# pyprob/pyprob

Measured on NVIDIA H100. Metric: ic_train_traces_per_sec, higher is better.
Workload: dtype f32

## Files before the change

### pyprob_b200/csrc/obs_embed.inc

```

struct ObsLayout {
  int in_off[PPB_MAX_OBS], out_off[PPB_MAX_OBS];
  int max_depth;
};
inline ObsLayout obs_layout(const ppb_net_desc& D) {
  ObsLayout o;
  int ci = 0, co = 0;
  o.max_depth = 0;
  for (int j = 0; j < D.num_obs; ++j) {
    o.in_off[j] = ci; o.out_off[j] = co;
    ci += D.obs_ff[j].in_dim; co += D.obs_ff[j].out_dim;
    o.max_depth = D.obs_ff[j].num_layers > o.max_depth ? D.obs_ff[j].num_layers : o.max_depth;
  }
  return o;
}

template <class W>
void obs_fp32_plan_fwd(Builder& bl, const ppb_net_desc& D, const float* arena, const float* obs, int B, const W& w,
                       float* obs_emb) {
  const int E = D.obs_dim;
  const ObsLayout o = obs_layout(D);
  for (int l = 0; l < o.max_depth; ++l) {
    bl.begin();
    for (int j = 0; j < D.num_obs; ++j) {
      const ppb_ff_desc& ff = D.obs_ff[j];
      if (l >= ff.num_layers) continue;
      const ppb_linear_desc& L = ff.layers[l];
      const float* X = l == 0 ? obs + o.in_off[j] : w.obs_act[j][l - 1];
      int64_t ldx = l == 0 ? D.obs_in_total : ff.layers[l - 1].out_dim;
      bool last = (l == ff.num_layers - 1);
      float* Y = last ? w.obs_cat + o.out_off[j] : w.obs_act[j][l];
      int64_t ldy = last ? E : L.out_dim;
      bl.add(linear_fwd(X, ldx, arena + L.w_off, L.in_dim, arena + L.b_off, Y, ldy, B, L.out_dim, L.in_dim, gemm::kRelu));
    }
  }
  for (int l = 0; l < D.obs_final.num_layers; ++l) {
    bl.begin();
    const ppb_linear_desc& L = D.obs_final.layers[l];
    const float* X = l == 0 ? w.obs_cat : w.fin_act[l - 1];
    bool last = (l == D.obs_final.num_layers - 1);
    float* Y = last ? obs_emb : w.fin_act[l];
    bl.add(linear_fwd(X, L.in_dim, arena + L.w_off, L.in_dim, arena + L.b_off, Y, L.out_dim, B, L.out_dim, L.in_dim, gemm::kRelu));
  }
}

inline int obs_bias_grad(const ppb_linear_desc& L, const float* dY, int64_t ld, int B, float* grad, cudaStream_t st) {
  k_colsum_gather<<<dim3((L.out_dim + 31) / 32, 8), 256, 0, st>>>(dY, ld, nullptr, B, L.out_dim, grad + L.b_off);
  PPB_LAUNCH_CHECK();
  return PPB_OK;
}

int obs_fp32_plan_bwd(Builder& bl, const ppb_net_desc& D, const float* arena, float* grad, const float* obs, int B,
                      const Ws& w) {
  const int E = D.obs_dim;
  const int first = (int)bl.phases.size();
  for (int l = D.obs_final.num_layers - 1; l >= 0; --l) {
    const ppb_linear_desc& L = D.obs_final.layers[l];
    const float* X = l == 0 ? w.obs_cat : w.fin_act[l - 1];
    float* dY = (l == D.obs_final.num_layers - 1) ? w.d_obs_emb : w.d_fin_act[l];
    float* dX = l == 0 ? w.d_obs_cat : w.d_fin_act[l - 1];
    bl.begin();
    bl.add(linear_dw(dY, L.out_dim, X, L.in_dim, grad + L.w_off, L.in_dim, B, L.out_dim, L.in_dim));
    Problem px = linear_dx(dY, L.out_dim, arena + L.w_off, L.in_dim, dX, L.in_dim, B, L.out_dim, L.in_dim, gemm::kMaskAux);
    px.aux = X; px.ld_aux = L.in_dim;
    bl.add(px);
  }
  const ObsLayout o = obs_layout(D);
  for (int l = o.max_depth - 1; l >= 0; --l) {
    bl.begin();
    for (int j = 0; j < D.num_obs; ++j) {
      const ppb_ff_desc& ff = D.obs_ff[j];
      if (l >= ff.num_layers) continue;
      const ppb_linear_desc& L = ff.layers[l];
      bool last = (l == ff.num_layers - 1);
      const float* X = l == 0 ? obs + o.in_off[j] : w.obs_act[j][l - 1];
      int64_t ldx = l == 0 ? D.obs_in_total : ff.layers[l - 1].out_dim;
      const float* dY = last ? w.d_obs_cat + o.out_off[j] : w.d_obs_act[j][l];
      int64_t lddy = last ? E : L.out_dim;
      bl.add(linear_dw(dY, lddy, X, ldx, grad + L.w_off, L.in_dim, B, L.out_dim, L.in_dim));
      if (l > 0) {
        Problem px = linear_dx(dY, lddy, arena + L.w_off, L.in_dim, w.d_obs_act[j][l - 1], ff.layers[l - 1].out_dim, B,
                               L.out_dim, L.in_dim, gemm::kMaskAux);
        px.aux = w.obs_act[j][l - 1]; px.ld_aux = ff.layers[l - 1].out_dim;
        bl.add(px);
      }
    }
  }
  return first;
}

int obs_fp32_bwd(const Builder& bl, int first, const Problem* dev, const ppb_net_desc& D, float* grad, int B, const Ws& w,
                 cudaStream_t st) {
  const int E = D.obs_dim;
  k_mask_nonpos<<<ew_grid((int64_t)B * E), 256, 0, st>>>(w.d_obs_emb, w.obs_emb, (int64_t)B * E);
  PPB_LAUNCH_CHECK();
  int ph = first, rc;
  for (int l = D.obs_final.num_layers - 1; l >= 0; --l) {
    const ppb_linear_desc& L = D.obs_final.layers[l];
    float* dY = (l == D.obs_final.num_layers - 1) ? w.d_obs_emb : w.d_fin_act[l];
    rc = obs_bias_grad(L, dY, L.out_dim, B, grad, st); if (rc) return rc;
    rc = run_phase(bl.phases[ph++], dev, st); if (rc) return rc;
  }
  const ObsLayout o = obs_layout(D);
  for (int l = o.max_depth - 1; l >= 0; --l) {
    for (int j = 0; j < D.num_obs; ++j) {
      const ppb_ff_desc& ff = D.obs_ff[j];
      if (l >= ff.num_layers) continue;
      const ppb_linear_desc& L = ff.layers[l];
      bool last = (l == ff.num_layers - 1);
      const float* dY = last ? w.d_obs_cat + o.out_off[j] : w.d_obs_act[j][l];
      rc = obs_bias_grad(L, dY, last ? E : L.out_dim, B, grad, st); if (rc) return rc;
    }
    rc = run_phase(bl.phases[ph++], dev, st); if (rc) return rc;
  }
  return PPB_OK;
}

inline obsmlp::Plan obs_plan_of(const ppb_net_desc& D, const Ws* w, const float* obs) {
  obsmlp::Plan P;
  memset(&P, 0, sizeof(P));
  const int E = D.obs_dim;
  const ObsLayout lay = obs_layout(D);
  P.E = E;
  int nf = 0;
  auto add_layer = [&](const ppb_linear_desc& L) -> obsmlp::Layer& {
    obsmlp::Layer& o = P.L[P.n_layers++];
    o.in_dim = L.in_dim; o.out_dim = L.out_dim; o.w_off = L.w_off; o.b_off = L.b_off;
    o.pitch = (L.in_dim & 3) ? L.in_dim : ((L.in_dim & 7) ? L.in_dim : L.in_dim + 4);
    o.sw = nf;
    nf += (L.out_dim * o.pitch + L.out_dim + 3) & ~3;
    o.part = P.part_floats;
    P.part_floats += L.out_dim * L.in_dim + L.out_dim;
    return o;
  };
  std::vector<int> first(D.num_obs);
  for (int j = 0; j < D.num_obs; ++j) {
    const ppb_ff_desc& ff = D.obs_ff[j];
    first[j] = P.n_layers;
    for (int l = 0; l < ff.num_layers; ++l) {
      obsmlp::Layer& o = add_layer(ff.layers[l]);
      o.xoff = P.A; P.A += o.in_dim;
      if (l + 1 < ff.num_layers) { o.dzoff = P.Dz; P.Dz += o.out_dim; }
      o.dxoff = l == 0 ? -1 : P.L[P.n_layers - 2].dzoff;
      o.x = l == 0 ? obs + lay.in_off[j] : (w ? w->obs_act[j][l - 1] : nullptr);
      o.ldx = l == 0 ? D.obs_in_total : ff.layers[l - 1].out_dim;
      if (l + 1 < ff.num_layers) { o.y = w ? w->obs_act[j][l] : nullptr; o.ldy = o.out_dim; }
    }
  }
  const int cat = P.A, dcat = P.Dz;
  P.A += E; P.Dz += E;
  for (int j = 0; j < D.num_obs; ++j) {
    obsmlp::Layer& o = P.L[first[j] + D.obs_ff[j].num_layers - 1];
    o.yoff = cat + lay.out_off[j]; o.dzoff = dcat + lay.out_off[j];
    o.y = w ? w->obs_cat + lay.out_off[j] : nullptr; o.ldy = E;
  }
  for (int j = 0; j < D.num_obs; ++j)
    for (int l = 0; l + 1 < D.obs_ff[j].num_layers; ++l) P.L[first[j] + l].yoff = P.L[first[j] + l + 1].xoff;
  const int nfin = D.obs_final.num_layers;
  for (int l = 0; l < nfin; ++l) {
    const bool last = l == nfin - 1;
    obsmlp::Layer& o = add_layer(D.obs_final.layers[l]);
    if (l == 0) o.xoff = cat;
    o.yoff = P.A; P.A += o.out_dim;
    o.dzoff = P.Dz; P.Dz += o.out_dim;
    o.dxoff = l == 0 ? dcat : P.L[P.n_layers - 2].dzoff;
    o.x = l == 0 ? (w ? w->obs_cat : nullptr) : (w ? w->fin_act[l - 1] : nullptr);
    o.ldx = o.in_dim;
    o.y = w ? (last ? w->obs_emb : w->fin_act[l]) : nullptr; o.ldy = o.out_dim;
    if (l > 0) o.xoff = P.L[P.n_layers - 2].yoff;
  }
  P.w_floats = nf;
  return P;
}
inline bool obs_fused_ok(const ppb_net_desc& D) {
  constexpr int kFuseMaxWidth = obsmlp::W2;
  if (D.obs_dim > kFuseMaxWidth) return false;
  for (int j = 0; j < D.num_obs; ++j)
    for (int l = 0; l < D.obs_ff[j].num_layers; ++l)
      if (D.obs_ff[j].layers[l].in_dim > kFuseMaxWidth || D.obs_ff[j].layers[l].out_dim > kFuseMaxWidth) return false;
  for (int l = 0; l < D.obs_final.num_layers; ++l)
    if (D.obs_final.layers[l].in_dim > kFuseMaxWidth || D.obs_final.layers[l].out_dim > kFuseMaxWidth) return false;
  const obsmlp::Plan P = obs_plan_of(D, nullptr, nullptr);
  return obsmlp::smem_fwd(P) <= obsmlp::kMaxSmem && obsmlp::smem_bwd(P) <= obsmlp::kMaxSmem;
}
int obs_fused_fwd(const ppb_net_desc& D, const float* arena, const float* obs, int B, const Ws& w, cudaStream_t st,
                  const HImg* emb_img = nullptr) {
  int rc = smem_opt_in<obsmlp::k_fwd>(obsmlp::kMaxSmem);
  if (rc) return rc;
  obsmlp::Plan P = obs_plan_of(D, &w, obs);
  if (emb_img) {
    P.emb_k_hi = emb_img->k_hi; P.emb_k_lo = emb_img->k_lo; P.emb_mn_hi = emb_img->mn_hi; P.emb_mn_lo = emb_img->mn_lo;
    P.emb_kb = emb_img->kb;
  }
  const int tpc = (B + PPB_NUM_SMS - 1) / PPB_NUM_SMS;
  PPB_CUDA(ppb_launch(obsmlp::k_fwd, dim3((B + tpc - 1) / tpc), dim3(obsmlp::kThreads), obsmlp::smem_fwd(P), st, 1, 0, P, arena,
                      B, tpc));
  PPB_LAUNCH_CHECK();
  return PPB_OK;
}
int obs_fused_bwd(const ppb_net_desc& D, const float* arena, float* grad, const float* obs, int B, const Ws& w,
                  cudaStream_t st) {
  int rc = smem_opt_in<obsmlp::k_bwd>(obsmlp::kMaxSmem);
  if (rc) return rc;
  const obsmlp::Plan P = obs_plan_of(D, &w, obs);
  constexpr int kMaxCtas = 16 * obsmlp::kCluster;
  int tpc = (B + kMaxCtas - 1) / kMaxCtas;
  tpc = tpc < obsmlp::kMT ? obsmlp::kMT : tpc;
  int ctas = (B + tpc - 1) / tpc;
  ctas = (ctas + obsmlp::kCluster - 1) / obsmlp::kCluster * obsmlp::kCluster;
  PPB_CUDA(ppb_launch(obsmlp::k_bwd, dim3(ctas), dim3(obsmlp::kThreads), obsmlp::smem_bwd(P), st, 1, obsmlp::kCluster, P, arena,
                      (const float*)w.d_obs_emb, grad, B, tpc));
  PPB_LAUNCH_CHECK();
  return PPB_OK;
}

inline bool obs_tc_ok(const ppb_net_desc& D) {
  const ObsLayout o = obs_layout(D);
  for (int j = 0; j < D.num_obs; ++j) {
    const ppb_ff_desc& ff = D.obs_ff[j];
    if (ff.num_layers < 2 || (o.out_off[j] & 31)) return false;
    for (int l = 1; l < ff.num_layers; ++l)
      if (ff.layers[l].in_dim < 32) return false;
  }
  for (int l = 0; l < D.obs_final.num_layers; ++l)
    if (D.obs_final.layers[l].in_dim < 32) return false;
  return true;
}

template <class Add>
void obs_weight_images(ppb_net* net, Add add) {
  const ppb_net_desc& D = net->desc;
  net->obs_form = obs_fused_ok(D) ? ObsForm::fused : obs_tc_ok(D) ? ObsForm::tensor_core : ObsForm::simt;
  if (net->obs_form != ObsForm::tensor_core) return;
  for (int j = 0; j < D.num_obs; ++j)
    for (int l = 1; l < D.obs_ff[j].num_layers; ++l) {
      const ppb_linear_desc& L = D.obs_ff[j].layers[l];
      net->w_obs[j][l] = add(L.w_off, L.out_dim, L.in_dim, L.in_dim);
    }
  for (int l = 0; l < D.obs_final.num_layers; ++l) {
    const ppb_linear_desc& L = D.obs_final.layers[l];
    net->w_fin[l] = add(L.w_off, L.out_dim, L.in_dim, L.in_dim);
  }
}

struct ObsImgs {
  HImg act[PPB_MAX_OBS][PPB_MAX_FF_LAYERS], cat, fin[PPB_MAX_FF_LAYERS];
  HImg g_act[PPB_MAX_OBS][PPB_MAX_FF_LAYERS], g_cat, g_fin[PPB_MAX_FF_LAYERS], g_emb;
  char* begin; int64_t bytes;
};
template <class Img>
void obs_carve_images(const ppb_net* net, int B, Img img, ObsImgs& o) {
  if (net->obs_form != ObsForm::tensor_core) return;
  const ppb_net_desc& D = net->desc;
  for (int j = 0; j < D.num_obs; ++j)
    for (int l = 0; l + 1 < D.obs_ff[j].num_layers; ++l) {
      o.act[j][l] = img(B, D.obs_ff[j].layers[l].out_dim);
      o.g_act[j][l] = img(B, D.obs_ff[j].layers[l].out_dim);
    }
  o.cat = img(B, D.obs_dim);
  o.g_cat = img(B, D.obs_dim);
  for (int l = 0; l + 1 < D.obs_final.num_layers; ++l) {
    o.fin[l] = img(B, D.obs_final.layers[l].out_dim);
    o.g_fin[l] = img(B, D.obs_final.layers[l].out_dim);
  }
  o.g_emb = img(B, D.obs_dim);
}

__global__ void __launch_bounds__(256) k_pack_rows_masked(float* __restrict__ g, const float* __restrict__ y, int rows,
                                                           int cols, int64_t ld, HImg img) {
  ppb_pdl_trigger();
  ppb_pdl_wait();
  tc::pack_tile<tc::Parts::both>(blockIdx.x, (int)img.kb, img.k_hi, img.k_lo, img.mn_hi, img.mn_lo,
                                 [&](int row, int k0, float (&x)[4]) {
#pragma unroll
    for (int j = 0; j < 4; ++j) {
      x[j] = 0.0f;
      if (row < rows && k0 + j < cols) {
        const int64_t o = (int64_t)row * ld + k0 + j;
        x[j] = y[o] > 0.0f ? g[o] : 0.0f;
        g[o] = x[j];
      }
    }
  });
}

struct ObsStep {
  Builder bl;
  std::vector<int> tc_ph;
  int tc_dw = -1;
};

int obs_plan_fwd(ppb_net* net, const float* arena, const ppb_batch* b, const Ws& w, const ObsImgs& im, const HImg& emb_img,
                 TcBuilder& tb, ObsStep& os, cudaStream_t st) {
  const ppb_net_desc& D = net->desc;
  const int B = b->n_traces, E = D.obs_dim;
  const ObsLayout o = obs_layout(D);
  if (net->obs_form == ObsForm::simt) obs_fp32_plan_fwd(os.bl, D, arena, b->obs, B, w, w.obs_emb);
  if (net->obs_form == ObsForm::tensor_core) {
    os.bl.begin();
    for (int j = 0; j < D.num_obs; ++j) {
      const ppb_linear_desc& L = D.obs_ff[j].layers[0];
      os.bl.add(linear_fwd(b->obs + o.in_off[j], D.obs_in_total, arena + L.w_off, L.in_dim, arena + L.b_off, w.obs_act[j][0],
                           L.out_dim, B, L.out_dim, L.in_dim, gemm::kRelu));
    }
  }
  int rc = upload_and_get(net, os.bl, w.problems, w.max_problems / 2, st, 0);
  if (rc) return rc;
  if (net->obs_form != ObsForm::tensor_core) return PPB_OK;
  auto add = [&](const ppb_linear_desc& L, const HImg& in, const WImg& wi, const HImg& out, int col0, float* c, int ldc) {
    tcg::Problem p = TP0();
    p.a = op_k(in.k_hi, in.k_lo, (int)in.kb, 0, 0);
    p.b = wk(net, wi);
    p.M = B; p.N = L.out_dim; p.K = L.in_dim;
    p.flags = tcg::kRelu; p.bias = arena + L.b_off;
    p.o_k_hi = out.k_hi; p.o_k_lo = out.k_lo; p.o_mn_hi = out.mn_hi; p.o_mn_lo = out.mn_lo;
    p.o_kb = (int)out.kb; p.o_row0 = 0; p.o_col0 = col0; p.c = c; p.ldc = ldc;
    tb.add(p);
  };
  for (int l = 1; l < o.max_depth; ++l) {
    os.tc_ph.push_back((int)tb.phases.size());
    tb.begin();
    for (int j = 0; j < D.num_obs; ++j) {
      const ppb_ff_desc& ff = D.obs_ff[j];
      if (l >= ff.num_layers) continue;
      const ppb_linear_desc& L = ff.layers[l];
      if (l == ff.num_layers - 1) add(L, im.act[j][l - 1], net->w_obs[j][l], im.cat, o.out_off[j], w.obs_cat + o.out_off[j], E);
      else add(L, im.act[j][l - 1], net->w_obs[j][l], im.act[j][l], 0, w.obs_act[j][l], L.out_dim);
    }
  }
  for (int l = 0; l < D.obs_final.num_layers; ++l) {
    const ppb_linear_desc& L = D.obs_final.layers[l];
    const HImg& in = l == 0 ? im.cat : im.fin[l - 1];
    os.tc_ph.push_back((int)tb.phases.size());
    tb.begin();
    if (l == D.obs_final.num_layers - 1) add(L, in, net->w_fin[l], emb_img, 0, w.obs_emb, L.out_dim);
    else add(L, in, net->w_fin[l], im.fin[l], 0, w.fin_act[l], L.out_dim);
  }
  return PPB_OK;
}

int obs_fwd(ppb_net* net, const float* arena, const ppb_batch* b, const Ws& w, const ObsImgs& im, const HImg& emb_img,
            const TcBuilder& tb, const tcg::Problem* tdev, const ObsStep& os, int precision, cudaStream_t st,
            cudaStream_t s_img) {
  const ppb_net_desc& D = net->desc;
  const int B = b->n_traces, E = D.obs_dim;
  int rc;
  const bool emb_packed = net->obs_form == ObsForm::fused && (B & 127) == 0 && (E & 31) == 0;
  if (net->obs_form == ObsForm::fused) { rc = obs_fused_fwd(D, arena, b->obs, B, w, st, emb_packed ? &emb_img : nullptr); if (rc) return rc; }
  if (net->obs_form == ObsForm::tensor_core && (B & 127))
    PPB_CUDA(cudaMemsetAsync(im.begin, 0, (size_t)im.bytes, st));
  for (const gemm::Phase& ph : os.bl.phases) { rc = run_phase(ph, w.problems, st); if (rc) return rc; }
  if (net->obs_form != ObsForm::tensor_core) {
    if (!emb_packed) {
      PPB_CUDA(ppb_launch(k_pack_rows, dim3(dim3((B + 127) / 128, 4)), dim3(256), 0, st, 1, 0, w.obs_emb, B, E, E, emb_img));
      PPB_LAUNCH_CHECK();
    }
    return stream_after(net, s_img, st);
  }
  for (int j = 0; j < D.num_obs; ++j) {
    const int od = D.obs_ff[j].layers[0].out_dim;
    PPB_CUDA(ppb_launch(k_pack_rows, dim3(dim3((B + 127) / 128, 4)), dim3(256), 0, st, 1, 0, w.obs_act[j][0], B, od, od, im.act[j][0]));
    PPB_LAUNCH_CHECK();
  }
  rc = stream_after(net, s_img, st); if (rc) return rc;
  for (int ph : os.tc_ph) { rc = run_tc_phase_auto<2>(tb.phases[ph], tdev, precision, st, tb); if (rc) return rc; }
  return PPB_OK;
}

int obs_plan_bwd(ppb_net* net, const float* arena, float* grad, const ppb_batch* b, const Ws& w, const ObsImgs& im,
                 TcBuilder& tb, ObsStep& os, cudaStream_t st) {
  const ppb_net_desc& D = net->desc;
  const int B = b->n_traces;
  const ObsLayout o = obs_layout(D);
  if (net->obs_form == ObsForm::simt) obs_fp32_plan_bwd(os.bl, D, arena, grad, b->obs, B, w);
  if (net->obs_form == ObsForm::tensor_core) {
    os.bl.begin();
    for (int j = 0; j < D.num_obs; ++j) {
      const ppb_linear_desc& L = D.obs_ff[j].layers[0];
      os.bl.add(linear_dw(w.d_obs_act[j][0], L.out_dim, b->obs + o.in_off[j], D.obs_in_total, grad + L.w_off, L.in_dim, B,
                          L.out_dim, L.in_dim));
    }
  }
  int rc = upload_and_get(net, os.bl, w.problems + w.max_problems / 2, w.max_problems / 2, st, 1);
  if (rc) return rc;
  if (net->obs_form != ObsForm::tensor_core) return PPB_OK;
  struct DwSpec { const HImg* gy; int gy_col0; const HImg* x; const ppb_linear_desc* L; };
  std::vector<DwSpec> dws;
  auto add_dx = [&](const ppb_linear_desc& L, const HImg& gy, int gy_col0, const WImg& wi, const HImg& x, float* c,
                    const HImg& gx) {
    tcg::Problem p = TP0();
    p.a = op_k(gy.k_hi, gy.k_lo, (int)gy.kb, 0, gy_col0);
    p.b = wmn(net, wi);
    p.M = B; p.N = L.in_dim; p.K = L.out_dim;
    p.flags = tcg::kMaskImg; p.mask_hi = x.k_hi;
    p.o_k_hi = gx.k_hi; p.o_k_lo = gx.k_lo; p.o_mn_hi = gx.mn_hi; p.o_mn_lo = gx.mn_lo;
    p.o_kb = (int)gx.kb; p.o_row0 = 0; p.o_col0 = 0; p.c = c; p.ldc = L.in_dim;
    tb.add(p);
    dws.push_back({&gy, gy_col0, &x, &L});
  };
  for (int l = D.obs_final.num_layers - 1; l >= 0; --l) {
    const ppb_linear_desc& L = D.obs_final.layers[l];
    os.tc_ph.push_back((int)tb.phases.size());
    tb.begin();
    add_dx(L, (l == D.obs_final.num_layers - 1) ? im.g_emb : im.g_fin[l], 0, net->w_fin[l], l == 0 ? im.cat : im.fin[l - 1],
           l == 0 ? w.d_obs_cat : w.d_fin_act[l - 1], l == 0 ? im.g_cat : im.g_fin[l - 1]);
  }
  for (int l = o.max_depth - 1; l >= 1; --l) {
    os.tc_ph.push_back((int)tb.phases.size());
    tb.begin();
    for (int j = 0; j < D.num_obs; ++j) {
      const ppb_ff_desc& ff = D.obs_ff[j];
      if (l >= ff.num_layers) continue;
      const bool last = l == ff.num_layers - 1;
      add_dx(ff.layers[l], last ? im.g_cat : im.g_act[j][l], last ? o.out_off[j] : 0, net->w_obs[j][l], im.act[j][l - 1],
             w.d_obs_act[j][l - 1], im.g_act[j][l - 1]);
    }
  }
  os.tc_dw = (int)tb.phases.size();
  tb.begin();
  int dw_tiles = 0;
  for (auto& s : dws) dw_tiles += ((s.L->out_dim + 127) / 128) * ((s.L->in_dim + 127) / 128);
  for (auto& s : dws) {
    tcg::Problem p = TP0();
    p.a = op_mn(s.gy->mn_hi, s.gy->mn_lo, (int)s.gy->kb, 0, s.gy_col0);
    p.b = op_mn(s.x->mn_hi, s.x->mn_lo, (int)s.x->kb, 0, 0);
    p.M = s.L->out_dim; p.N = s.L->in_dim; p.K = pad128(B);
    p.c = grad + s.L->w_off; p.ldc = s.L->in_dim;
    p.k_splits = pick_splits(p.M, p.N, p.K, dw_tiles);
    tb.add(p);
  }
  return PPB_OK;
}

int obs_bwd(ppb_net* net, const float* arena, float* grad, const ppb_batch* b, const Ws& w, const ObsImgs& im,
            const TcBuilder& tb, const tcg::Problem* tdev, const ObsStep& os, int precision, cudaStream_t st) {
  const ppb_net_desc& D = net->desc;
  const int B = b->n_traces, E = D.obs_dim;
  const Problem* dev = w.problems + w.max_problems / 2;
  if (net->obs_form == ObsForm::fused) return obs_fused_bwd(D, arena, grad, b->obs, B, w, st);
  if (net->obs_form == ObsForm::simt) return obs_fp32_bwd(os.bl, 0, dev, D, grad, B, w, st);
  PPB_CUDA(ppb_launch(k_pack_rows_masked, dim3(dim3((B + 127) / 128, 4)), dim3(256), 0, st, 1, 0, w.d_obs_emb, w.obs_emb, B, E, E, im.g_emb));
  PPB_LAUNCH_CHECK();
  int rc;
  for (int ph : os.tc_ph) { rc = run_tc_phase_auto<2>(tb.phases[ph], tdev, precision, st, tb); if (rc) return rc; }
  rc = run_tc_phase<1>(tb.phases[os.tc_dw], tdev, precision, st); if (rc) return rc;
  for (int l = 0; l < D.obs_final.num_layers; ++l) {
    const ppb_linear_desc& L = D.obs_final.layers[l];
    const float* dY = (l == D.obs_final.num_layers - 1) ? w.d_obs_emb : w.d_fin_act[l];
    rc = obs_bias_grad(L, dY, L.out_dim, B, grad, st); if (rc) return rc;
  }
  const ObsLayout o = obs_layout(D);
  for (int j = 0; j < D.num_obs; ++j) {
    const ppb_ff_desc& ff = D.obs_ff[j];
    for (int l = 0; l < ff.num_layers; ++l) {
      const ppb_linear_desc& L = ff.layers[l];
      const bool last = l == ff.num_layers - 1;
      const float* dY = last ? w.d_obs_cat + o.out_off[j] : w.d_obs_act[j][l];
      rc = obs_bias_grad(L, dY, last ? E : L.out_dim, B, grad, st); if (rc) return rc;
    }
  }
  return run_phase(os.bl.phases[0], dev, st);
}
```

### pyprob_b200/csrc/obs_mlp.cuh

```cuda
#pragma once
#include "common.cuh"
#include "tc.cuh"
#include "tc_cluster.cuh"

namespace obsmlp {

constexpr int W2 = 96;
constexpr int kThreads = 256;
constexpr int kSlices = 8;
constexpr int kRows = kThreads / kSlices;
constexpr int kMT = 4;
constexpr int kCluster = 8;
constexpr int kMaxLayers = PPB_MAX_OBS * PPB_MAX_FF_LAYERS + PPB_MAX_FF_LAYERS;
constexpr size_t kMaxSmem = 227 * 1024;

struct Layer {
  int in_dim, out_dim;
  int sw, pitch;
  int xoff, yoff;
  int dzoff, dxoff;
  int part;
  int64_t w_off, b_off;
  float* y; int ldy;
  const float* x; int ldx;
};

struct Plan {
  int n_layers;
  int A, Dz;
  int w_floats, part_floats;
  int E;
  Layer L[kMaxLayers];
  float* emb_k_hi; float* emb_k_lo; float* emb_mn_hi; float* emb_mn_lo;
  long long emb_kb;
};

inline size_t smem_fwd(const Plan& p) { return (size_t)(p.w_floats + kMT * p.A) * sizeof(float); }
inline size_t smem_bwd(const Plan& p) { return (size_t)(p.w_floats + p.part_floats + kMT * (p.A + p.Dz)) * sizeof(float); }

__device__ __forceinline__ void cp_async16(float* smem_dst, const float* gmem_src) {
  asm volatile("cp.async.cg.shared.global [%0], [%1], 16;" ::"r"((uint32_t)__cvta_generic_to_shared(smem_dst)), "l"(gmem_src)
               : "memory");
}
__device__ __forceinline__ void cp_async4(float* smem_dst, const float* gmem_src) {
  asm volatile("cp.async.ca.shared.global [%0], [%1], 4;" ::"r"((uint32_t)__cvta_generic_to_shared(smem_dst)), "l"(gmem_src)
               : "memory");
}
__device__ __forceinline__ void cp_async_wait_all() {
  asm volatile("cp.async.commit_group;" ::: "memory");
  asm volatile("cp.async.wait_group 0;" ::: "memory");
}

__device__ __forceinline__ void stage_layer(float* smem, const float* __restrict__ arena, const Layer& L) {
  const int in_dim = L.in_dim, out_dim = L.out_dim, pitch = L.pitch;
  float* dst = smem + L.sw;
  const float* src = arena + L.w_off;
  const float* bsrc = arena + L.b_off;
  if ((in_dim & 3) == 0) {
    const int q = in_dim >> 2, nq = out_dim * q;
    for (int c = threadIdx.x; c < nq; c += kThreads) {
      const int n = c / q, k4 = c - n * q;
      cp_async16(dst + n * pitch + 4 * k4, src + 4 * c);
    }
  } else {
    const int nw = out_dim * in_dim;
    for (int c = threadIdx.x; c < nw; c += kThreads) cp_async4(dst + c, src + c);
  }
  float* bias = dst + out_dim * pitch;
  for (int n = threadIdx.x; n < out_dim; n += kThreads) cp_async4(bias + n, bsrc + n);
}
__device__ __forceinline__ void load_rows(float* dst, int pitch, const float* src, int64_t ld, int tr0, int nt, int width) {
  for (int idx = threadIdx.x; idx < nt * width; idx += kThreads) {
    const int t = idx / width, k = idx - t * width;
    cp_async4(dst + t * pitch + k, src + (int64_t)(tr0 + t) * ld + k);
  }
}

__device__ __forceinline__ float group_sum(float v) {
  v += __shfl_xor_sync(0xffffffffu, v, 4);
  v += __shfl_xor_sync(0xffffffffu, v, 2);
  v += __shfl_xor_sync(0xffffffffu, v, 1);
  return v;
}
__device__ __forceinline__ float pick(const float (&a)[kMT], int i) {
  float r = a[0];
#pragma unroll
  for (int t = 1; t < kMT; ++t) r = i == t ? a[t] : r;
  return r;
}

__device__ __forceinline__ void layer_fwd(const Plan& P, const Layer& L, const float* smem, float* act, int tr0, int nt,
                                          bool last) {
  const int g = threadIdx.x / kSlices, s = threadIdx.x % kSlices;
  const int in_dim = L.in_dim, out_dim = L.out_dim, pitch = L.pitch, A = P.A, ldy = L.ldy;
  const float* w = smem + L.sw;
  const float* bias = w + out_dim * pitch;
  const float* xr = act + L.xoff;
  float* yr = act + L.yoff;
  float* y = L.y;
  float* ek_hi = last ? P.emb_k_hi : nullptr;
  float* ek_lo = P.emb_k_lo;
  float* em_hi = P.emb_mn_hi;
  float* em_lo = P.emb_mn_lo;
  const long long kb = P.emb_kb;
  for (int n = g; n - (g & 3) < out_dim; n += kRows) {
    float acc[kMT];
#pragma unroll
    for (int t = 0; t < kMT; ++t) acc[t] = 0.f;
    const float* wr = w + n * pitch;
    const int kend = n < out_dim ? in_dim : 0;
    for (int k = s; k < kend; k += kSlices) {
      const float wv = wr[k];
#pragma unroll
      for (int t = 0; t < kMT; ++t) acc[t] = fmaf(wv, xr[t * A + k], acc[t]);
    }
#pragma unroll
    for (int t = 0; t < kMT; ++t) acc[t] = group_sum(acc[t]);
    if (s < nt && n < out_dim) {
      const float v = fmaxf(pick(acc, s) + bias[n], 0.f);
      const int tr = tr0 + s;
      yr[s * A + n] = v;
      y[(int64_t)tr * ldy + n] = v;
      if (ek_hi) {
        float hi, lo;
        tc::split_tf32(v, hi, lo);
        const int64_t ok = tc::packed_offset(tr, n, kb);
        ek_hi[ok] = hi;
        if (ek_lo) ek_lo[ok] = lo;
        if (em_hi) {
          const int64_t om = tc::packed_offset_mn(tr, n, kb);
          em_hi[om] = hi;
          if (em_lo) em_lo[om] = lo;
        }
      }
    }
  }
}

__global__ void __launch_bounds__(kThreads) k_fwd(const __grid_constant__ Plan P, const float* __restrict__ arena, int B,
                                                  int traces_per_cta) {
  ppb_pdl_wait();
  ppb_pdl_trigger();
  extern __shared__ __align__(16) float smem[];
  const int n_layers = P.n_layers, A = P.A;
  float* act = smem + P.w_floats;
  for (int i = 0; i < n_layers; ++i) stage_layer(smem, arena, P.L[i]);
  const int t_begin = blockIdx.x * traces_per_cta;
  const int t_end = min(B, t_begin + traces_per_cta);
  for (int c0 = t_begin; c0 < t_end; c0 += kMT) {
    const int nt = min(kMT, t_end - c0);
    for (int i = 0; i < n_layers; ++i) {
      const Layer& L = P.L[i];
      if (L.dxoff < 0) load_rows(act + L.xoff, A, L.x, L.ldx, c0, nt, L.in_dim);
    }
    cp_async_wait_all();
    __syncthreads();
    for (int i = 0; i < n_layers; ++i) {
      layer_fwd(P, P.L[i], smem, act, c0, nt, i == n_layers - 1);
      __syncthreads();
    }
  }
}

__device__ __forceinline__ void layer_dx(const Plan& P, const Layer& L, const float* smem, const float* act, float* dz,
                                         int nt) {
  const int g = threadIdx.x / kSlices, s = threadIdx.x % kSlices;
  const int in_dim = L.in_dim, out_dim = L.out_dim, pitch = L.pitch, A = P.A, Dz = P.Dz;
  const float* w = smem + L.sw;
  const float* dr = dz + L.dzoff;
  const float* xr = act + L.xoff;
  float* dxr = dz + L.dxoff;
  for (int k = g; k - (g & 3) < in_dim; k += kRows) {
    float acc[kMT];
#pragma unroll
    for (int t = 0; t < kMT; ++t) acc[t] = 0.f;
    const int nend = k < in_dim ? out_dim : 0;
    for (int n = s; n < nend; n += kSlices) {
      const float wv = w[n * pitch + k];
#pragma unroll
      for (int t = 0; t < kMT; ++t) acc[t] = fmaf(wv, dr[t * Dz + n], acc[t]);
    }
#pragma unroll
    for (int t = 0; t < kMT; ++t) acc[t] = group_sum(acc[t]);
    if (s < nt && k < in_dim) dxr[s * Dz + k] = xr[s * A + k] > 0.f ? pick(acc, s) : 0.f;
  }
}

__device__ __forceinline__ void layer_partial(const Plan& P, const Layer& L, const float* act, const float* dz, float* part,
                                              int nt) {
  const int in_dim = L.in_dim, out_dim = L.out_dim, A = P.A, Dz = P.Dz;
  const int nw = out_dim * in_dim;
  const float* dr = dz + L.dzoff;
  const float* xr = act + L.xoff;
  float* pr = part + L.part;
  for (int e = threadIdx.x; e < nw + out_dim; e += kThreads) {
    float v = 0.f;
    if (e < nw) {
      const int n = e / in_dim, k = e - n * in_dim;
#pragma unroll
      for (int t = 0; t < kMT; ++t)
        if (t < nt) v = fmaf(dr[t * Dz + n], xr[t * A + k], v);
    } else {
#pragma unroll
      for (int t = 0; t < kMT; ++t)
        if (t < nt) v += dr[t * Dz + e - nw];
    }
    pr[e] += v;
  }
}

__global__ void __launch_bounds__(kThreads) k_bwd(const __grid_constant__ Plan P, const float* __restrict__ arena,
                                                  const float* __restrict__ d_emb, float* __restrict__ grad, int B,
                                                  int traces_per_cta) {
  ppb_pdl_trigger();
  extern __shared__ __align__(16) float smem[];
  const int n_layers = P.n_layers, A = P.A, Dz = P.Dz, E = P.E, part_floats = P.part_floats;
  float* act = smem + P.w_floats;
  float* dz = act + kMT * A;
  float* part = dz + kMT * Dz;
  for (int i = 0; i < n_layers; ++i)
    if (P.L[i].dxoff >= 0) stage_layer(smem, arena, P.L[i]);
  for (int i = threadIdx.x; i < part_floats; i += kThreads) part[i] = 0.f;
  ppb_pdl_wait();
  const int t_begin = blockIdx.x * traces_per_cta;
  const int t_end = min(B, t_begin + traces_per_cta);
  const int zoff = P.L[n_layers - 1].dzoff, eoff = P.L[n_layers - 1].yoff;
  const float* emb = P.L[n_layers - 1].y;
  for (int c0 = t_begin; c0 < t_end; c0 += kMT) {
    const int nt = min(kMT, t_end - c0);
    for (int i = 0; i < n_layers; ++i) {
      const Layer& L = P.L[i];
      load_rows(act + L.xoff, A, L.x, L.ldx, c0, nt, L.in_dim);
    }
    load_rows(act + eoff, A, emb, E, c0, nt, E);
    load_rows(dz + zoff, Dz, d_emb, E, c0, nt, E);
    cp_async_wait_all();
    __syncthreads();
    for (int idx = threadIdx.x; idx < nt * E; idx += kThreads) {
      const int t = idx / E, k = idx - t * E;
      if (!(act[t * A + eoff + k] > 0.f)) dz[t * Dz + zoff + k] = 0.f;
    }
    __syncthreads();
    for (int i = n_layers - 1; i >= 0; --i) {
      if (P.L[i].dxoff < 0) continue;
      layer_dx(P, P.L[i], smem, act, dz, nt);
      __syncthreads();
    }
    for (int i = 0; i < n_layers; ++i) layer_partial(P, P.L[i], act, dz, part, nt);
    __syncthreads();
  }
  cp_async_wait_all();
  tcc::cluster_sync_all();
  const uint32_t rank = tcc::cluster_ctarank();
  const uint32_t part_addr = (uint32_t)__cvta_generic_to_shared(part);
  int li = 0, lpart = P.L[0].part, lnext = n_layers > 1 ? P.L[1].part : part_floats, lnw = P.L[0].out_dim * P.L[0].in_dim;
  int64_t lw = P.L[0].w_off, lb = P.L[0].b_off;
  for (int e = rank * kThreads + threadIdx.x; e < part_floats; e += kCluster * kThreads) {
    float v = 0.f;
#pragma unroll
    for (int r = 0; r < kCluster; ++r) v += tcc::ld_cluster(tcc::map_to_rank(part_addr + 4u * (uint32_t)e, (uint32_t)r));
    while (e >= lnext) {
      ++li;
      const Layer& L = P.L[li];
      lpart = L.part; lnw = L.out_dim * L.in_dim; lw = L.w_off; lb = L.b_off;
      lnext = li + 1 < n_layers ? P.L[li + 1].part : part_floats;
    }
    const int le = e - lpart;
    if (v != 0.f) atomicAdd(grad + (le < lnw ? lw + le : lb + (le - lnw)), v);
  }
  tcc::cluster_sync_all();
}

}
```

Before: 1.646 million.

## Drop cluster DSMEM reduction in obs backward; use 64 independent CTAs

Removes the 8-CTA cluster launch and the distributed shared-memory cross-CTA reduction of weight-gradient partials. Each CTA now atomically adds its own partials to global memory, and the grid is capped at 64 CTAs with traces per CTA rounded to multiples of kMT. The per-layer partial loop is also split into a weight pass with incremental index stepping (no per-element divide) and a separate bias pass. The trade-off is more global atomics per gradient element, in exchange for dropping cluster syncs and cluster scheduling constraints and getting fewer, larger CTAs.

```diff
diff --git a/pyprob_b200/csrc/obs_embed.inc b/pyprob_b200/csrc/obs_embed.inc
--- a/pyprob_b200/csrc/obs_embed.inc
+++ b/pyprob_b200/csrc/obs_embed.inc
@@ -198,17 +198,17 @@
   PPB_LAUNCH_CHECK();
   return PPB_OK;
 }
+inline int obs_fused_bwd_tpc(int B) {
+  const int chunks = (B + obsmlp::kMT - 1) / obsmlp::kMT;
+  return (chunks + obsmlp::kBwdMaxCtas - 1) / obsmlp::kBwdMaxCtas * obsmlp::kMT;
+}
 int obs_fused_bwd(const ppb_net_desc& D, const float* arena, float* grad, const float* obs, int B, const Ws& w,
                   cudaStream_t st) {
   int rc = smem_opt_in<obsmlp::k_bwd>(obsmlp::kMaxSmem);
   if (rc) return rc;
   const obsmlp::Plan P = obs_plan_of(D, &w, obs);
-  constexpr int kMaxCtas = 16 * obsmlp::kCluster;
-  int tpc = (B + kMaxCtas - 1) / kMaxCtas;
-  tpc = tpc < obsmlp::kMT ? obsmlp::kMT : tpc;
-  int ctas = (B + tpc - 1) / tpc;
-  ctas = (ctas + obsmlp::kCluster - 1) / obsmlp::kCluster * obsmlp::kCluster;
-  PPB_CUDA(ppb_launch(obsmlp::k_bwd, dim3(ctas), dim3(obsmlp::kThreads), obsmlp::smem_bwd(P), st, 1, obsmlp::kCluster, P, arena,
+  const int tpc = obs_fused_bwd_tpc(B);
+  PPB_CUDA(ppb_launch(obsmlp::k_bwd, dim3((B + tpc - 1) / tpc), dim3(obsmlp::kThreads), obsmlp::smem_bwd(P), st, 1, 0, P, arena,
                       (const float*)w.d_obs_emb, grad, B, tpc));
   PPB_LAUNCH_CHECK();
   return PPB_OK;
diff --git a/pyprob_b200/csrc/obs_mlp.cuh b/pyprob_b200/csrc/obs_mlp.cuh
--- a/pyprob_b200/csrc/obs_mlp.cuh
+++ b/pyprob_b200/csrc/obs_mlp.cuh
@@ -1,7 +1,6 @@
 #pragma once
 #include "common.cuh"
 #include "tc.cuh"
-#include "tc_cluster.cuh"
 
 namespace obsmlp {
 
@@ -10,7 +9,7 @@
 constexpr int kSlices = 8;
 constexpr int kRows = kThreads / kSlices;
 constexpr int kMT = 4;
-constexpr int kCluster = 8;
+constexpr int kBwdMaxCtas = 64;
 constexpr int kMaxLayers = PPB_MAX_OBS * PPB_MAX_FF_LAYERS + PPB_MAX_FF_LAYERS;
 constexpr size_t kMaxSmem = 227 * 1024;
 
@@ -193,19 +192,27 @@
   const float* dr = dz + L.dzoff;
   const float* xr = act + L.xoff;
   float* pr = part + L.part;
-  for (int e = threadIdx.x; e < nw + out_dim; e += kThreads) {
+  const int dn = kThreads / in_dim, dk = kThreads - dn * in_dim;
+  int n = threadIdx.x / in_dim, k = threadIdx.x - n * in_dim;
+  for (int e = threadIdx.x; e < nw; e += kThreads) {
     float v = 0.f;
-    if (e < nw) {
-      const int n = e / in_dim, k = e - n * in_dim;
-#pragma unroll
-      for (int t = 0; t < kMT; ++t)
-        if (t < nt) v = fmaf(dr[t * Dz + n], xr[t * A + k], v);
-    } else {
-#pragma unroll
-      for (int t = 0; t < kMT; ++t)
-        if (t < nt) v += dr[t * Dz + e - nw];
+#pragma unroll
+    for (int t = 0; t < kMT; ++t) {
+      const float d = dr[t * Dz + n], x = xr[t * A + k];
+      v = t < nt ? fmaf(d, x, v) : v;
     }
     pr[e] += v;
+    n += dn; k += dk;
+    if (k >= in_dim) { k -= in_dim; ++n; }
+  }
+  for (int j = threadIdx.x; j < out_dim; j += kThreads) {
+    float v = 0.f;
+#pragma unroll
+    for (int t = 0; t < kMT; ++t) {
+      const float d = dr[t * Dz + j];
+      v = t < nt ? v + d : v;
+    }
+    pr[nw + j] += v;
   }
 }
 
@@ -250,15 +257,10 @@
     __syncthreads();
   }
   cp_async_wait_all();
-  tcc::cluster_sync_all();
-  const uint32_t rank = tcc::cluster_ctarank();
-  const uint32_t part_addr = (uint32_t)__cvta_generic_to_shared(part);
   int li = 0, lpart = P.L[0].part, lnext = n_layers > 1 ? P.L[1].part : part_floats, lnw = P.L[0].out_dim * P.L[0].in_dim;
   int64_t lw = P.L[0].w_off, lb = P.L[0].b_off;
-  for (int e = rank * kThreads + threadIdx.x; e < part_floats; e += kCluster * kThreads) {
-    float v = 0.f;
-#pragma unroll
-    for (int r = 0; r < kCluster; ++r) v += tcc::ld_cluster(tcc::map_to_rank(part_addr + 4u * (uint32_t)e, (uint32_t)r));
+  for (int e = threadIdx.x; e < part_floats; e += kThreads) {
+    const float v = part[e];
     while (e >= lnext) {
       ++li;
       const Layer& L = P.L[li];
@@ -268,7 +270,6 @@
     const int le = e - lpart;
     if (v != 0.f) atomicAdd(grad + (le < lnw ? lw + le : lb + (le - lnw)), v);
   }
-  tcc::cluster_sync_all();
-}
-
-}
+}
+
+}
```

Measured after the change: 1.692 million, median of 6. 2.8% higher.
